# AberHu/TF-NAS

Hardware: AMD Instinct MI355X
Metric: supernet search images/sec (w-step + alpha-step) (higher is better)
Workload: dtype fp32

## Files before the change

tf-nas_amd/csrc/dwconv_kernels.hip:

```cpp
#include <cstring>
#include <type_traits>
#include "tfnas_dev.h"
#include "kernels.h"
#include "prof.h"
#include "efree.h"

__device__ __forceinline__ int floordiv(int a, int b) { return a >= 0 ? a / b : -((-a + b - 1) / b); }

__device__ __forceinline__ int xcd_first_tile() {
    const int gx = gridDim.x, bx = blockIdx.x;
    return (gx & 7) ? bx : (bx & 7) * (gx >> 3) + (bx >> 3);
}

template <int K, int DIL = 0>
__device__ __forceinline__ bool dw_locate(const TfnasCellDesc& d, int cy, int CC, int& g, int& c0) {
    for (g = 0; g < d.G; ++g) {
        if (d.g[g].k != K) continue;
        if (DIL != 0 && group_dil(d, g) != DIL) continue;
        const int t = (d.g[g].mcp + CC - 1) / CC;
        if (cy < t) {
            c0 = cy * CC;
            return true;
        }
        cy -= t;
    }
    return false;
}

struct DwSeg {
    int g, c0, mc, mcp, cs, woff;
};
template <int K, int DIL>
__device__ __forceinline__ bool dw_locate_seg(const TfnasCellDesc& d, int cy, int CC, DwSeg& sg) {
    for (int g = 0; g < d.G; ++g) {
        if (group_dil(d, g) != DIL) continue;
        const int n = group_nseg(d, g), q = d.g[g].mcp >> 2, mc = d.g[g].mc;
        int woff = 0;
        for (int s = 0; s < n; ++s) {
            const int ks = seg_k(d, g, s), lo = 4 * seg_quad0(q, n, s), hi = 4 * seg_quad0(q, n, s + 1);
            const int top = hi < mc ? hi : mc;
            if (ks == K) {
                const int t = (hi - lo + CC - 1) / CC;
                if (cy < t) {
                    sg = DwSeg{g, lo + cy * CC, top, hi, lo, woff};
                    return true;
                }
                cy -= t;
            }
            woff += (top - lo) * ks * ks;
        }
    }
    return false;
}

__device__ __forceinline__ void dw_flush_pair(f32x4 a, f32x4 b, float* red, int CC, int c0, int mcp, float* acc,
                                              bool = false) {
    const int tid = threadIdx.x, CQ = CC >> 2;
    __syncthreads();
    st4(red + tid * 8, a);
    st4(red + tid * 8 + 4, b);
    __syncthreads();
    if (tid < CC && c0 + tid < mcp) {
        const int cq = tid >> 2, comp = tid & 3;
        float s = 0.f, q = 0.f;
        for (int t = cq; t < 256; t += CQ) {
            s += red[t * 8 + comp];
            q += red[t * 8 + 4 + comp];
        }
        acc[2 * (size_t)(c0 + tid) + 0] = s;
        acc[2 * (size_t)(c0 + tid) + 1] = q;
    }
}

__device__ __forceinline__ void dw_flush_stats(f32x4 a, f32x4 b, float* lds, int CC, int c0, int mcp, int off, int M, float* part,
                                               int lane) {
    dw_flush_pair(a, b, lds, CC, c0, mcp, part + (size_t)lane * 2 * M + 2 * (size_t)off);
}

__device__ __forceinline__ void stage_weights(float* wts, const float* __restrict__ w, int KK, int CC, int c0, int mc, int cs = 0) {
    for (int idx = threadIdx.x; idx < KK * CC; idx += 256) {
        const int cl = idx % CC, t = idx / CC;
        wts[t * CC + cl] = (c0 + cl < mc) ? w[(size_t)(c0 + cl - cs) * KK + t] : 0.f;
    }
}

template <class FAddr, class FXf>
__device__ __forceinline__ void load_tile2(float* tile, int L0, int L1, int CC, int cq_shift,
                                           const float* __restrict__ src0, const float* __restrict__ src1, FAddr addr,
                                           FXf xf) {
    const int CQ = CC >> 2, total = L0 * L1 * CQ;
    const float inv_l1 = 1.f / (float)L1;
    for (int base = 0; base < total; base += 1024) {
        f32x4 v0[4], v1[4];
        int pix[4], cqv[4];
        bool ok[4];
#pragma unroll
        for (int u = 0; u < 4; ++u) {
            const int idx = base + u * 256 + threadIdx.x;
            pix[u] = idx >> cq_shift;
            cqv[u] = idx & (CQ - 1);
            const int r = (int)(((float)pix[u] + 0.5f) * inv_l1);
            const int c = pix[u] - r * L1;
            size_t a = 0;
            ok[u] = idx < total && addr(r, c, cqv[u], a);
            v0[u] = ok[u] ? ld4_nt(src0 + a) : zero4();
            v1[u] = ok[u] ? ld4_nt(src1 + a) : zero4();
        }
#pragma unroll
        for (int u = 0; u < 4; ++u) {
            const int idx = base + u * 256 + threadIdx.x;
            if (idx < total) st4(tile + pix[u] * CC + 4 * cqv[u], ok[u] ? xf(v0[u], v1[u], cqv[u]) : zero4());
        }
    }
}

template <class FAddr, class FXf>
__device__ __forceinline__ void load_tile(float* tile, int L0, int L1, int CC, int cq_shift, const float* __restrict__ src,
                                          FAddr addr, FXf xf) {
    const int CQ = CC >> 2, total = L0 * L1 * CQ;
    const float inv_l1 = 1.f / (float)L1;
    for (int base = 0; base < total; base += 1024) {
        f32x4 v[4];
        int pix[4], cqv[4];
        bool ok[4];
#pragma unroll
        for (int u = 0; u < 4; ++u) {
            const int idx = base + u * 256 + threadIdx.x;
            pix[u] = idx >> cq_shift;
            cqv[u] = idx & (CQ - 1);
            const int r = (int)(((float)pix[u] + 0.5f) * inv_l1);
            const int c = pix[u] - r * L1;
            size_t a = 0;
            ok[u] = idx < total && addr(r, c, cqv[u], a);
            v[u] = ok[u] ? ld4_nt(src + a) : zero4();
        }
#pragma unroll
        for (int u = 0; u < 4; ++u) {
            const int idx = base + u * 256 + threadIdx.x;
            if (idx < total) st4(tile + pix[u] * CC + 4 * cqv[u], ok[u] ? xf(v[u], cqv[u]) : zero4());
        }
    }
}

template <int K, int S, int ACT, int KQ, bool RAW = false, int DIL = 1>
__global__ __launch_bounds__(256, 4) void k_dw_fwd(TfnasCellDesc d, const float* __restrict__ E,
                                                   const float* __restrict__ x,
                                                   const double* __restrict__ stats1, float* __restrict__ D,
                                                   float* __restrict__ part, DwGeom gm) {
    extern __shared__ __attribute__((aligned(16))) float lds[];
    int g, c0, lane = blockIdx.x, cy = blockIdx.y;
    static_assert(DIL == 1 || (DIL == 2 && KQ == 0 && (K == 3 || K == 5)), "dilation 2: 3 x 3 / 5 x 5 from E or raw x");
    if (KQ > 0) efree_lane_chunk(lane, cy);
    DwSeg sg;
    if constexpr (KQ > 0) {
        if (!dw_locate<K, DIL>(d, cy, gm.CC, g, c0)) return;
        sg = DwSeg{g, c0, d.g[g].mc, d.g[g].mcp, 0, 0};
    } else {
        if (!dw_locate_seg<K, DIL>(d, cy, gm.CC, sg)) return;
        g = sg.g, c0 = sg.c0;
    }
    const int mc = sg.mc, mcp = sg.mcp, off = d.g[g].off;
    const int CC = gm.CC, CQ = CC >> 2, TH = gm.T0, TW = gm.T1;
    const int H = d.H, W = d.W, Ho = d.Ho, Wo = d.Wo, M = d.M;
    const int tid = threadIdx.x;
    const int IH = gm.L0, IW = gm.L1;

    const int tile_floats = max(IH * IW * CC, 2048);
    float* in_tile = lds;
    float* wts = lds + tile_floats;
    float2* cst = reinterpret_cast<float2*>(wts + K * K * CC);

    if constexpr (!RAW) {
    if (tid < CC)
        cst[tid] = (c0 + tid < mc) ? bn_consts(stats1 + 2 * (size_t)(off + c0 + tid), 1.0 / ((double)d.N * H * W), d.eps)
                                   : make_float2(0.f, 0.f);
    }
    stage_weights(wts, d.g[g].w_dw + sg.woff, K * K, CC, c0, mc, sg.cs);
    ExpandB<(KQ > 0 ? KQ : 2)> xb;
    if (KQ > 0) {
        __syncthreads();
        expand_b_load(xb, d.g[g].w_expand, d.ic, c0, mc, cst);
    }

    constexpr int KE = DIL * (K - 1) + 1, WIN = 3 * S + KE;
    const int nsw = TW >> 2, nstrips = TH * nsw;
    f32x4 ssum = zero4(), ssq = zero4();
    for (int t = KQ > 0 ? lane : xcd_first_tile(); t < gm.ntiles; t += gridDim.x) {
        const int tw = t % gm.tilesW, th = (t / gm.tilesW) % gm.tilesH, n = t / (gm.tilesW * gm.tilesH);
        const int ho0 = th * TH, wo0 = tw * TW;
        const int hi0 = ho0 * S - DIL * (K / 2), wi0 = wo0 * S - DIL * (K / 2);
        __syncthreads();
        if (KQ > 0) {
            const float inv_iw = 1.f / (float)IW;
            expand_tile<(KQ > 0 ? KQ : 2), ACT>(in_tile, IH * IW, CC, x, xb, [&](int p, size_t& a) {
                const int r = (int)(((float)p + 0.5f) * inv_iw), c = p - r * IW;
                const int hi = hi0 + r, wi = wi0 + c;
                a = ((size_t)(n * H + hi) * W + wi) * d.ic;
                return hi >= 0 && hi < H && wi >= 0 && wi < W;
            });
        } else if constexpr (RAW) {
            load_tile(in_tile, IH, IW, CC, gm.cq_shift, x,
                      [&](int r, int c, int cq, size_t& a) {
                          const int hi = hi0 + r, wi = wi0 + c;
                          a = ((size_t)(n * H + hi) * W + wi) * d.ic + c0 + 4 * cq;
                          return hi >= 0 && hi < H && wi >= 0 && wi < W && c0 + 4 * cq < mcp;
                      },
                      [&](f32x4 v, int) { return v; });
        } else
        load_tile(in_tile, IH, IW, CC, gm.cq_shift, E,
                  [&](int r, int c, int cq, size_t& a) {
                      const int hi = hi0 + r, wi = wi0 + c;
                      a = ((size_t)(n * H + hi) * W + wi) * M + off + c0 + 4 * cq;
                      return hi >= 0 && hi < H && wi >= 0 && wi < W && c0 + 4 * cq < mcp;
                  },
                  [&](f32x4 v, int cq) {
#pragma unroll
                      for (int j = 0; j < 4; ++j) {
                          const float2 c = cst[4 * cq + j];
                          v[j] = act_f<ACT>((v[j] - c.x) * c.y);
                      }
                      return v;
                  });
        __syncthreads();
        for (int item = tid; item < nstrips * CQ; item += 256) {
            const int cq = item & (CQ - 1), st = item >> gm.cq_shift;
            const int oh = st / nsw, ow0 = (st - oh * nsw) * 4;
            f32x4 acc[4] = {zero4(), zero4(), zero4(), zero4()};
#pragma unroll 1
            for (int ky = 0; ky < K; ++ky) {
                const float* rowp = in_tile + ((oh * S + ky * DIL) * IW + ow0 * S) * CC + 4 * cq;
                const float* wp = wts + ky * K * CC + 4 * cq;
                f32x4 win[WIN];
#pragma unroll
                for (int u = 0; u < WIN; ++u) win[u] = ld4(rowp + u * CC);
#pragma unroll
                for (int kx = 0; kx < K; ++kx) {
                    const f32x4 wv = ld4(wp + kx * CC);
#pragma unroll
                    for (int j = 0; j < 4; ++j) acc[j] += win[j * S + kx * DIL] * wv;
                }
            }
            const int ho = ho0 + oh;
            if (ho < Ho && c0 + 4 * cq < mcp) {
#pragma unroll
                for (int j = 0; j < 4; ++j) {
                    const int wo = wo0 + ow0 + j;
                    if (wo < Wo) {
                        st4_nt(D + (((size_t)(n * Ho + ho) * Wo + wo) * M + off + c0 + 4 * cq), acc[j]);
                        ssum += acc[j];
                        ssq += acc[j] * acc[j];
                    }
                }
            }
        }
    }
    dw_flush_stats(ssum, ssq, in_tile, CC, c0, mcp, off, M, part, lane);
}


template <int K, int S, int ACT, int KQ, bool RAW = false, int DIL = 1>
__global__ __launch_bounds__(256, 4) void k_dw_bwd_data(TfnasCellDesc d, const float* __restrict__ dZ,
                                                        const float* __restrict__ gate, const float* __restrict__ dpooled,
                                                        const float* __restrict__ D, const double* __restrict__ stats2,
                                                        const double* __restrict__ red2, const float* __restrict__ E,
                                                        const float* __restrict__ x,
                                                        const double* __restrict__ stats1, float* __restrict__ dEh,
                                                        float* __restrict__ part, DwGeom gm, int dx_accum) {
    extern __shared__ __attribute__((aligned(16))) float lds[];
    int g, c0, lane = blockIdx.x, cy = blockIdx.y;
    static_assert(DIL == 1 || (DIL == 2 && KQ == 0 && (K == 3 || K == 5)), "dilation 2: 3 x 3 / 5 x 5 from E or raw x");
    if (KQ > 0) efree_lane_chunk(lane, cy);
    DwSeg sg;
    if constexpr (KQ > 0) {
        if (!dw_locate<K, DIL>(d, cy, gm.CC, g, c0)) return;
        sg = DwSeg{g, c0, d.g[g].mc, d.g[g].mcp, 0, 0};
    } else {
        if (!dw_locate_seg<K, DIL>(d, cy, gm.CC, sg)) return;
        g = sg.g, c0 = sg.c0;
    }
    const int mc = sg.mc, mcp = sg.mcp, off = d.g[g].off;
    const int CC = gm.CC, CQ = CC >> 2, TIH = gm.T0, TIW = gm.T1;
    const int H = d.H, W = d.W, Ho = d.Ho, Wo = d.Wo, M = d.M;
    constexpr int PAD = DIL * (K / 2), KE = DIL * (K - 1) + 1;
    const int tid = threadIdx.x;
    const int OH = gm.L0, OW = gm.L1;

    const int tile_floats = max(OH * OW * CC, 2048);
    float* dd_tile = lds;
    float* wts = lds + tile_floats;
    f32x4* cst2 = reinterpret_cast<f32x4*>(wts + K * K * CC);
    float2* cst1 = reinterpret_cast<float2*>(cst2 + CC);

    fill_cst2(cst2, d, CC, c0, mc, off, stats2, red2);
    if constexpr (!RAW) {
    if (tid < CC)
        cst1[tid] = (c0 + tid < mc) ? bn_consts(stats1 + 2 * (size_t)(off + c0 + tid), 1.0 / ((double)d.N * H * W), d.eps)
                                    : make_float2(0.f, 0.f);
    }
    stage_weights(wts, d.g[g].w_dw + sg.woff, K * K, CC, c0, mc, sg.cs);
    float* eh_tile = reinterpret_cast<float*>(cst1 + CC);
    ExpandB<(KQ > 0 ? KQ : 2)> xb;
    if (KQ > 0) {
        __syncthreads();
        expand_b_load(xb, d.g[g].w_expand, d.ic, c0, mc, cst1);
    }

    const int nsw = TIW >> 2, nstrips = TIH * nsw;
    const bool has_se = d.g[g].se > 0;
    const float inv_hw = 1.f / (float)(Ho * Wo);
    f32x4 t1 = zero4(), t2 = zero4();
    for (int t = KQ > 0 ? lane : xcd_first_tile(); t < gm.ntiles; t += gridDim.x) {
        const int tw = t % gm.tilesW, th = (t / gm.tilesW) % gm.tilesH, n = t / (gm.tilesW * gm.tilesH);
        const int hi0 = th * TIH, wi0 = tw * TIW;
        const int oh0 = floordiv(hi0 + PAD - (KE - 1), S), ow0 = floordiv(wi0 + PAD - (KE - 1), S);
        __syncthreads();
        const int mycq = tid & (CQ - 1);
        f32x4 g4 = zero4(), dp4 = zero4();
        if (has_se && c0 + 4 * mycq < mcp) {
            g4 = ld4(gate + (size_t)n * M + off + c0 + 4 * mycq);
            dp4 = ld4(dpooled + (size_t)n * M + off + c0 + 4 * mycq) * splat4(inv_hw);
        }
        load_tile2(dd_tile, OH, OW, CC, gm.cq_shift, dZ, D,
                   [&](int r, int c, int cq, size_t& a) {
                       const int ho = oh0 + r, wo = ow0 + c;
                       a = ((size_t)(n * Ho + ho) * Wo + wo) * M + off + c0 + 4 * cq;
                       return ho >= 0 && ho < Ho && wo >= 0 && wo < Wo && c0 + 4 * cq < mcp;
                   },
                   [&](f32x4 v, f32x4 dv, int cq) { return bn2_dd<ACT>(cst2, 4 * cq, v, dv, has_se, g4, dp4); });
        if (KQ > 0) {
            const float inv_iw = 1.f / (float)TIW;
            expand_tile<(KQ > 0 ? KQ : 2), 2>(eh_tile, TIH * TIW, CC, x, xb, [&](int p, size_t& a) {
                const int r = (int)(((float)p + 0.5f) * inv_iw), c = p - r * TIW;
                const int hi = hi0 + r, wi = wi0 + c;
                a = ((size_t)(n * H + hi) * W + wi) * d.ic;
                return hi < H && wi < W;
            });
        }
        __syncthreads();

        for (int item = tid; item < nstrips * CQ; item += 256) {
            const int cq = item & (CQ - 1), st = item >> gm.cq_shift;
            const int ihp = st / nsw, iw0 = (st - ihp * nsw) * 4;
            const int half = (TIH + 1) >> 1;
            const int ih = (S == 2) ? (ihp < half ? 2 * ihp : 2 * (ihp - half) + 1) : ihp;
            const int hi = hi0 + ih;
            f32x4 acc[4] = {zero4(), zero4(), zero4(), zero4()};
            f32x4 ev[4];
#pragma unroll
            for (int j = 0; j < 4; ++j) {
                const int wi = wi0 + iw0 + j;
                const bool okj = hi < H && wi < W && c0 + 4 * cq < mcp;
                if constexpr (RAW) {
                    const size_t a = ((size_t)(n * H + hi) * W + wi) * d.ic + c0 + 4 * cq;
                    ev[j] = (okj && x) ? ld4_nt(x + a) : zero4();
                    if (okj && dx_accum) ev[j] += ld4_nt(dEh + a);
                }
                else if (KQ > 0) ev[j] = ld4(eh_tile + (ih * TIW + iw0 + j) * CC + 4 * cq);
                else ev[j] = okj ? ld4_nt(E + (((size_t)(n * H + hi) * W + wi) * M + off + c0 + 4 * cq)) : zero4();
            }
            if (S == 1) {
#pragma unroll 1
                for (int ky = 0; ky < K; ++ky) {
                    const int r = hi + PAD - ky * DIL - oh0;
                    const float* rowp = dd_tile + (r * OW + iw0) * CC + 4 * cq;
                    const float* wp = wts + ky * K * CC + 4 * cq;
                    f32x4 win[KE + 3];
#pragma unroll
                    for (int u = 0; u < KE + 3; ++u) win[u] = ld4(rowp + u * CC);
#pragma unroll
                    for (int kx = 0; kx < K; ++kx) {
                        const f32x4 wv = ld4(wp + kx * CC);
#pragma unroll
                        for (int j = 0; j < 4; ++j) acc[j] += win[j - kx * DIL + KE - 1] * wv;
                    }
                }
            } else {
                const int base = wi0 + iw0;
#pragma unroll 1
                for (int ky = 0; ky < K; ++ky) {
                    const int tt = hi + PAD - ky * DIL;
                    if (tt & 1) continue;
                    const int r = tt / 2 - oh0;
                    const float* wp = wts + ky * K * CC + 4 * cq;
#pragma unroll
                    for (int kx = 0; kx < K; ++kx) {
                        const f32x4 wv = ld4(wp + kx * CC);
#pragma unroll
                        for (int j = 0; j < 4; ++j) {
                            if ((j + PAD - kx * DIL) & 1) continue;
                            const int c = base / 2 + (j + PAD - kx * DIL) / 2 - ow0;
                            acc[j] += ld4(dd_tile + (r * OW + c) * CC + 4 * cq) * wv;
                        }
                    }
                }
            }
            if (hi < H && c0 + 4 * cq < mcp) {
#pragma unroll
                for (int j = 0; j < 4; ++j) {
                    const int wi = wi0 + iw0 + j;
                    if (wi < W) {
                        if constexpr (RAW) {
                            st4_nt(dEh + (((size_t)(n * H + hi) * W + wi) * d.ic + c0 + 4 * cq), acc[j] + ev[j]);
                        } else {
                        const size_t a = ((size_t)(n * H + hi) * W + wi) * M + off + c0 + 4 * cq;
                        const f32x4 e = ev[j];
                        f32x4 deh;
#pragma unroll
                        for (int q = 0; q < 4; ++q) {
                            const float2 c = cst1[4 * cq + q];
                            const float eh = KQ > 0 ? e[q] : (e[q] - c.x) * c.y;
                            deh[q] = acc[j][q] * act_d<ACT>(eh);
                            t1[q] += deh[q];
                            t2[q] += deh[q] * eh;
                        }
                        st4_nt(dEh + a, deh);
                        }
                    }
                }
            }
        }
    }
    if constexpr (!RAW) dw_flush_stats(t1, t2, dd_tile, CC, c0, mcp, off, M, part, lane);
}

template <int K, int S, int ACT, int KY0, int KR, bool RAW, int DIL>
__device__ __forceinline__ void dw_wgrad_rows(const TfnasCellDesc& d, const float* __restrict__ dZ,
                                              const float* __restrict__ gate, const float* __restrict__ dpooled,
                                              const float* __restrict__ D, const double* __restrict__ stats2,
                                              const double* __restrict__ red2, const float* __restrict__ E,
                                              const double* __restrict__ stats1, float* __restrict__ part,
                                              size_t out_size, const DwGeom& gm) {
    extern __shared__ __attribute__((aligned(16))) float lds[];
    DwSeg sg;
    if (!dw_locate_seg<K, DIL>(d, blockIdx.y, gm.CC, sg)) return;
    const int g = sg.g, c0 = sg.c0;
    const int mc = sg.mc, mcp = sg.mcp, off = d.g[g].off;
    size_t poff = sg.woff;
    for (int gg = 0; gg < g; ++gg) poff += group_dw_floats(d, gg);
    float* __restrict__ gw = part + (size_t)blockIdx.x * out_size + poff;
    const int CC = gm.CC, CQ = CC >> 2, TH = gm.T0, TW = gm.T1;
    const int H = d.H, W = d.W, Ho = d.Ho, Wo = d.Wo, M = d.M;
    const int tid = threadIdx.x;
    const int IH = gm.L0, IW = gm.L1;

    const int tile_floats = max(IH * IW * CC, 4 * KR * K * CC);
    float* in_tile = lds;
    f32x4* cst2 = reinterpret_cast<f32x4*>(lds + tile_floats);
    float2* cst1 = reinterpret_cast<float2*>(cst2 + CC);

    fill_cst2(cst2, d, CC, c0, mc, off, stats2, red2);
    if constexpr (!RAW) {
    if (tid < CC)
        cst1[tid] = (c0 + tid < mc) ? bn_consts(stats1 + 2 * (size_t)(off + c0 + tid), 1.0 / ((double)d.N * H * W), d.eps)
                                    : make_float2(0.f, 0.f);
    }

    constexpr int KE = DIL * (K - 1) + 1, WIN = 3 * S + KE;
    const int nsw = TW >> 2, nstrips = TH * nsw;
    const bool has_se = d.g[g].se > 0;
    const float inv_hw = 1.f / (float)(Ho * Wo);
    f32x4 wacc[KR * K];
#pragma unroll
    for (int u = 0; u < KR * K; ++u) wacc[u] = zero4();
    for (int t = xcd_first_tile(); t < gm.ntiles; t += gridDim.x) {
        const int tw = t % gm.tilesW, th = (t / gm.tilesW) % gm.tilesH, n = t / (gm.tilesW * gm.tilesH);
        const int ho0 = th * TH, wo0 = tw * TW;
        const int hi0 = ho0 * S - DIL * (K / 2), wi0 = wo0 * S - DIL * (K / 2);
        const int mycq = tid & (CQ - 1);
        f32x4 g4 = zero4(), dp4 = zero4();
        if (has_se && c0 + 4 * mycq < mcp) {
            g4 = ld4(gate + (size_t)n * M + off + c0 + 4 * mycq);
            dp4 = ld4(dpooled + (size_t)n * M + off + c0 + 4 * mycq) * splat4(inv_hw);
        }
        const int nitems = nstrips * CQ;
        auto item_ops = [&](int item, f32x4 (&dd)[4], f32x4 (&dv)[4], bool (&ok)[4]) {
            const int cq = item & (CQ - 1), st = item >> gm.cq_shift;
            const int oh = st / nsw, ow0 = (st - oh * nsw) * 4;
            const int ho = ho0 + oh;
#pragma unroll
            for (int j = 0; j < 4; ++j) {
                const int wo = wo0 + ow0 + j;
                ok[j] = ho < Ho && wo < Wo && c0 + 4 * cq < mcp;
                const size_t a = ((size_t)(n * Ho + ho) * Wo + wo) * M + off + c0 + 4 * cq;
                dd[j] = ok[j] ? ld4_nt(dZ + a) : zero4();
                dv[j] = ok[j] ? ld4_nt(D + a) : zero4();
            }
        };
        constexpr bool PF = KR == K;
        f32x4 pdd[PF ? 4 : 1], pdv[PF ? 4 : 1];
// ... 354 lines not shown
        return p;
    }
    dw_tile_plan(d, d.Ho, d.Wo, true, 2048, wout, false, p);
    return p;
}

template <bool TILE, int... Vs, class F>
static bool dw_dispatch_k(int k, int stride, int act, int v, F&& f) {
    bool hit = false;
    auto with_v = [&](auto K, auto S, auto A) {
        ((v == Vs ? (f(K, S, A, std::integral_constant<int, Vs>{}), hit = true) : false) || ...);
    };
    auto with_a = [&](auto K, auto S) {
        if (act == TFNAS_ACT_RELU) with_v(K, S, std::integral_constant<int, TFNAS_ACT_RELU>{});
        else if (act == TFNAS_ACT_SWISH) with_v(K, S, std::integral_constant<int, TFNAS_ACT_SWISH>{});
        else if constexpr (TILE) {
            if (act == TFNAS_ACT_RELU6) with_v(K, S, std::integral_constant<int, TFNAS_ACT_RELU6>{});
            else if (act == TFNAS_ACT_HSWISH) with_v(K, S, std::integral_constant<int, TFNAS_ACT_HSWISH>{});
        }
    };
    auto with_s = [&](auto K) {
        if (stride == 1) with_a(K, std::integral_constant<int, 1>{});
        else with_a(K, std::integral_constant<int, 2>{});
    };
    if (k == 3) with_s(std::integral_constant<int, 3>{});
    else if (k == 5) with_s(std::integral_constant<int, 5>{});
    else if constexpr (TILE) {
        if (k == 7) with_s(std::integral_constant<int, 7>{});
    }
    return hit;
}
template <int... Vs, class F>
static bool dw_dispatch(int k, int stride, int act, int v, F&& f) {
    return dw_dispatch_k<false, Vs...>(k, stride, act, v, f);
}
template <int... Vs, class F>
static bool dw_tile_dispatch(int k, int stride, int act, int v, F&& f) {
    return dw_dispatch_k<true, Vs...>(k, stride, act, v, f);
}
template <int... Vs, class F>
static bool dw_tile_dispatch_d(int k, int dil, int stride, int act, int v, F&& f) {
    if (dil == 1)
        return dw_tile_dispatch<Vs...>(k, stride, act, v, [&](auto K, auto S, auto A, auto V) {
            f(K, S, A, V, std::integral_constant<int, 1>{});
        });
    if (dil != 2 || (k != 3 && k != 5) || v != 0) return false;
    return dw_tile_dispatch<0>(k, stride, act, 0, [&](auto K, auto S, auto A, auto V) {
        if constexpr (K != 7) f(K, S, A, V, std::integral_constant<int, 2>{});
    });
}
constexpr int DW_WG = -1;
static int dws_variant(const DwPlan& p) { return p.fuse_wgrad ? DW_WG : p.kq ? p.kq : (int)p.pipe; }

static int dw_reduce_wgrad(const TfnasCellDesc& d, const float* wpart, int rows, size_t wout, hipStream_t s) {
    size_t poff = 0;
    for (int g = 0; g < d.G; ++g) {
        const int n = (int)group_dw_floats(d, g);
        const int rc = launch_reduce_rows(wpart + poff, rows, n, wout, nullptr, d.g[g].g_dw, s, wgrad_accum(d));
        if (rc) return rc;
        poff += n;
    }
    return 0;
}

int launch_dw_fwd(const TfnasCellDesc& d, const float* E, const float* x, const double* stats1, float* D,
                  double* stats2, float* part, hipStream_t s) {
    const bool raw = cell_noexpand(d);
    if (raw ? !x : (!E && (!efree_ic_ok(d.ic) || dw_tile_only(d)))) return TFNAS_EINVAL;
    const DwPlan p = dw_plan_fwd(d, !raw && E == nullptr, x != nullptr);
    for (int i = 0; i < DW_NK; ++i) {
        if (!p.chunks[i]) continue;
        const int kk = dw_slot_k(i), dil = dw_slot_dil(i);
        ProfScope _prof(TK_DW_FWD, s, d.G > 2);
        bool ok = false;
        if (p.fam != DW_TILE && i >= 2) return TFNAS_EINVAL;
        if (p.fam == DW_DIRECT) {
            const DwDirect gm = p.direct[i];
            ok = dw_dispatch<2, 4>(kk, d.stride, d.act, p.jw, [&](auto K, auto S, auto A, auto JW) {
                hipLaunchKernelGGL((k_dwd_fwd<K, S, A, JW>), dim3(gm.nwg), dim3(256), 0, s, d, E, stats1, D, part, gm);
            });
        } else if (p.fam == DW_RING) {
            const DwSlide gm = p.ring[i];
            const size_t shm = (size_t)(gm.RB * gm.L1 * gm.CCP + kk * kk * gm.CC + 2 * gm.CC) * sizeof(float);
            ok = dw_dispatch<0, 1, 6, 10>(kk, d.stride, d.act, dws_variant(p), [&](auto K, auto, auto A, auto V) {
                hipLaunchKernelGGL((k_dws_fwd<K, A, V == 1, V == 1 ? 0 : V>), dim3(p.rows * gm.chunks), dim3(256), shm, s, d, E,
                                   stats1, D, part, gm, V > 1 ? x : nullptr);
            });
        } else {
            const DwGeom gm = p.tile[i];
            const int tile = gm.L0 * gm.L1 * gm.CC > 2048 ? gm.L0 * gm.L1 * gm.CC : 2048;
            const size_t shm = (size_t)(tile + kk * kk * gm.CC + 2 * gm.CC) * sizeof(float);
            if (shm > 64 * 1024) return TFNAS_ERANGE;
            if (raw)
                ok = dw_tile_dispatch_d<0>(kk, dil, d.stride, TFNAS_ACT_RELU, 0, [&](auto K, auto S, auto, auto, auto DIL) {
                    hipLaunchKernelGGL((k_dw_fwd<K, S, TFNAS_ACT_RELU, 0, true, DIL>), dim3(p.rows, p.chunks[i]), dim3(256), shm, s,
                                       d, nullptr, x, nullptr, D, part, gm);
                });
            else
            ok = dw_tile_dispatch_d<0, 4, 6, 10>(kk, dil, d.stride, d.act, p.kq, [&](auto K, auto S, auto A, auto KQ, auto DIL) {
                if constexpr ((K != 7 && !act_tile_only(A)) || KQ == 0)
                    hipLaunchKernelGGL((k_dw_fwd<K, S, A, KQ, false, DIL>), dim3(p.rows, p.chunks[i]), dim3(256), shm, s, d, E, x,
                                       stats1, D, part, gm);
            });
        }
        if (!ok) return TFNAS_EINVAL;
    }
    return reduce_pair_rows(d, part, p.rows, stats2, s);
}

int launch_dw_bwd_data(const DwPlan& p, const TfnasCellDesc& d, const float* dZ, const float* gate, const float* dpooled,
                       const float* D, const double* stats2, const double* red2, const float* E, const float* x,
                       const double* stats1, float* dEh, double* red1, float* part, hipStream_t s, float* cb1) {
    if (cell_noexpand(d)) return TFNAS_EINVAL;
    if (!E && (!efree_ic_ok(d.ic) || dw_tile_only(d))) return TFNAS_EINVAL;
    const size_t wout = dw_wout_size(d);
    float* wpart = part + (((size_t)p.rows * 2 * d.M + 63) & ~(size_t)63);
    for (int i = 0; i < DW_NK; ++i) {
        if (!p.chunks[i]) continue;
        const int kk = dw_slot_k(i), dil = dw_slot_dil(i);
        ProfScope _prof(TK_DW_BWD_DATA, s, d.G > 2);
        bool ok = false;
        if (p.fam != DW_TILE && i >= 2) return TFNAS_EINVAL;
        if (p.fam == DW_DIRECT) {
            const DwDirect gm = p.direct[i];
            ok = dw_dispatch<2, 4, DW_WG>(kk, d.stride, d.act, p.fuse_wgrad ? DW_WG : p.jw, [&](auto K, auto S, auto A, auto V) {
                if constexpr (V == DW_WG)
                    hipLaunchKernelGGL((k_dwd_bwd<K, 2, A, 2, true>), dim3(gm.nwg), dim3(256), 0, s, d, dZ, gate, dpooled, D,
                                       stats2, red2, E, stats1, dEh, part, gm, wpart, wout);
                else
                    hipLaunchKernelGGL((k_dwd_bwd<K, S, A, V>), dim3(gm.nwg), dim3(256), 0, s, d, dZ, gate, dpooled, D, stats2,
                                       red2, E, stats1, dEh, part, gm);
            });
        } else if (p.fam == DW_RING) {
            const DwSlide gm = p.ring[i];
            size_t shm = (size_t)(gm.RB * gm.L1 * gm.CCP + kk * kk * gm.CC + 4 * gm.CC + 2 * gm.CC +
                                  (p.kq ? gm.TH * gm.TW * gm.CCP : 0)) * sizeof(float);
            if (p.fuse_wgrad && shm < (size_t)4 * kk * kk * gm.CC * sizeof(float)) shm = (size_t)4 * kk * kk * gm.CC * sizeof(float);
            ok = dw_dispatch<0, 1, 6, 10, DW_WG>(kk, d.stride, d.act, dws_variant(p), [&](auto K, auto, auto A, auto V) {
                if constexpr (V == DW_WG) {
                    if constexpr (K == 3)
                        hipLaunchKernelGGL((k_dws_bwd<K, A, false, 0, true>), dim3(p.rows * gm.chunks), dim3(256), shm, s, d, dZ,
                                           gate, dpooled, D, stats2, red2, E, stats1, dEh, part, gm, nullptr, wpart, wout);
                } else {
                    hipLaunchKernelGGL((k_dws_bwd<K, A, V == 1, V == 1 ? 0 : V>), dim3(p.rows * gm.chunks), dim3(256), shm, s, d,
                                       dZ, gate, dpooled, D, stats2, red2, E, stats1, dEh, part, gm, V > 1 ? x : nullptr);
                }
            });
        } else {
            const DwGeom gm = p.tile[i];
            const int tile = gm.L0 * gm.L1 * gm.CC > 2048 ? gm.L0 * gm.L1 * gm.CC : 2048;
            const size_t shm = (size_t)(tile + kk * kk * gm.CC + 4 * gm.CC + 2 * gm.CC + (p.kq ? gm.T0 * gm.T1 * gm.CC : 0)) *
                               sizeof(float);
            if (shm > 64 * 1024) return TFNAS_ERANGE;
            ok = dw_tile_dispatch_d<0, 4, 6, 10>(kk, dil, d.stride, d.act, p.kq, [&](auto K, auto S, auto A, auto KQ, auto DIL) {
                if constexpr ((K != 7 && !act_tile_only(A)) || KQ == 0)
                    hipLaunchKernelGGL((k_dw_bwd_data<K, S, A, KQ, false, DIL>), dim3(p.rows, p.chunks[i]), dim3(256), shm, s, d, dZ,
                                       gate, dpooled, D, stats2, red2, E, x, stats1, dEh, part, gm, 0);
            });
        }
        if (!ok) return TFNAS_EINVAL;
    }
    if (p.fuse_wgrad) {
        ProfScope _prof(TK_DW_WGRAD, s);
        const int rc = dw_reduce_wgrad(d, wpart, p.rows, wout, s);
        if (rc) return rc;
    }
    if (cb1) return launch_reduce_bn1(d, part, p.rows, stats1, red1, cb1, s);
    return launch_reduce_rows(part, p.rows, 2 * d.M, 2 * (size_t)d.M, red1, nullptr, s);
}

int launch_dw_bwd_dx(const TfnasCellDesc& d, const float* dZ, const float* gate, const float* dpooled, const float* D,
                     const double* stats2, const double* red2, const float* dres, float* dx, hipStream_t s, bool accum) {
    if (!cell_noexpand(d) || !dx) return TFNAS_EINVAL;
    if (accum && d.G != 1) return TFNAS_EINVAL;
    const DwPlan p = dw_plan_bwd_data(d, false, false);
    if (p.fam != DW_TILE) return TFNAS_EINVAL;
    for (int i = 0; i < DW_NK; ++i) {
        if (!p.chunks[i]) continue;
        const int kk = dw_slot_k(i), dil = dw_slot_dil(i);
        ProfScope _prof(TK_DW_BWD_DATA, s, false);
        const DwGeom gm = p.tile[i];
        const int tile = gm.L0 * gm.L1 * gm.CC > 2048 ? gm.L0 * gm.L1 * gm.CC : 2048;
        const size_t shm = (size_t)(tile + kk * kk * gm.CC + 4 * gm.CC + 2 * gm.CC) * sizeof(float);
        if (shm > 64 * 1024) return TFNAS_ERANGE;
        const bool ok = dw_tile_dispatch_d<0>(kk, dil, d.stride, d.act, 0, [&](auto K, auto S, auto A, auto, auto DIL) {
            hipLaunchKernelGGL((k_dw_bwd_data<K, S, A, 0, true, DIL>), dim3(p.rows, p.chunks[i]), dim3(256), shm, s, d, dZ, gate,
                               dpooled, D, stats2, red2, nullptr, dres, nullptr, dx, nullptr, gm, (int)accum);
        });
        if (!ok) return TFNAS_EINVAL;
    }
    return (int)hipGetLastError();
}

static constexpr int dw_wgrad_kr(int k, int stride, int dil) { return k == 7 ? 4 : (k == 5 && dil == 2 && stride == 1) ? 3 : k; }

int launch_dw_wgrad(const TfnasCellDesc& d, const float* dZ, const float* gate, const float* dpooled, const float* D,
                    const double* stats2, const double* red2, const float* E, const double* stats1, float* part,
                    hipStream_t s) {
    if (!dw_wgrad_row_fits(d)) return TFNAS_ERANGE;
    const DwPlan p = dw_plan_wgrad(d);
    const size_t wout = dw_wout_size(d);
    for (int i = 0; i < DW_NK; ++i) {
        if (!p.chunks[i]) continue;
        const int kk = dw_slot_k(i), dil = dw_slot_dil(i);
        ProfScope _prof(TK_DW_WGRAD, s);
        if (p.fam != DW_TILE && i >= 2) return TFNAS_EINVAL;
        if (p.fam == DW_DIRECT) {
            const DwDirect gm = p.direct[i];
            dw_dispatch<2, 4>(kk, d.stride, d.act, p.jw, [&](auto K, auto S, auto A, auto JW) {
                hipLaunchKernelGGL((k_dwd_wgrad<K, S, A, JW>), dim3(gm.nwg), dim3(256), 0, s, d, dZ, gate, dpooled, D, stats2,
                                   red2, E, stats1, part, wout, gm);
            });
        } else if (p.fam == DW_RING) {
            const DwSlide gm = p.ring[i];
            int ring = gm.RB * gm.L1 * gm.CCP;
            if (ring < 4 * kk * kk * gm.CC) ring = 4 * kk * kk * gm.CC;
            const size_t shm = (size_t)(ring + 4 * gm.CC + 2 * gm.CC) * sizeof(float);
            dw_dispatch<0, 1>(kk, d.stride, d.act, p.pipe, [&](auto K, auto, auto A, auto PIPE) {
                hipLaunchKernelGGL((k_dws_wgrad<K, A, PIPE == 1>), dim3(p.rows * gm.chunks), dim3(256), shm, s, d, dZ, gate,
                                   dpooled, D, stats2, red2, E, stats1, part, wout, gm);
            });
        } else {
            const DwGeom gm = p.tile[i];
            const int kr = dw_wgrad_kr(kk, d.stride, dil);
            int tile = gm.L0 * gm.L1 * gm.CC;
            if (tile < 4 * kr * kk * gm.CC) tile = 4 * kr * kk * gm.CC;
            const size_t shm = (size_t)(tile + 4 * gm.CC + 2 * gm.CC) * sizeof(float);
            if (shm > 64 * 1024) return TFNAS_ERANGE;
            if (cell_noexpand(d))
                dw_tile_dispatch_d<0>(kk, dil, d.stride, d.act, 0, [&](auto K, auto S, auto A, auto, auto DIL) {
                    constexpr int KR = dw_wgrad_kr(K, S, DIL);
                    hipLaunchKernelGGL((k_dw_wgrad<K, S, A, KR, true, DIL>), dim3(p.rows, p.chunks[i], (K + KR - 1) / KR), dim3(256),
                                       shm, s, d, dZ, gate, dpooled, D, stats2, red2, E, nullptr, part, wout, gm);
                });
            else
            dw_tile_dispatch_d<0>(kk, dil, d.stride, d.act, 0, [&](auto K, auto S, auto A, auto, auto DIL) {
                constexpr int KR = dw_wgrad_kr(K, S, DIL);
                hipLaunchKernelGGL((k_dw_wgrad<K, S, A, KR, false, DIL>), dim3(p.rows, p.chunks[i], (K + KR - 1) / KR), dim3(256), shm,
                                   s, d, dZ, gate, dpooled, D, stats2, red2, E, stats1, part, wout, gm);
            });
        }
    }
    const int rc = dw_reduce_wgrad(d, part, p.rows, wout, s);
    return rc ? rc : (int)hipGetLastError();
}
```

tf-nas_amd/csrc/efree.h:

```cpp
#pragma once
#include "tfnas_dev.h"

template <int KQ>
struct ExpandB {
    float b[2][KQ];
    float2 bc[2];
};

template <int KQ>
__device__ __forceinline__ void expand_b_load(ExpandB<KQ>& B, const float* __restrict__ w_expand, int ic, int c0, int mc,
                                              const float2* cst) {
    const int lane = threadIdx.x & 63, n = lane & 15, q = lane >> 4;
#pragma unroll
    for (int nt = 0; nt < 2; ++nt) {
        const int ch = c0 + 16 * nt + n;
#pragma unroll
        for (int kk = 0; kk < KQ; kk += 2) {
            float2 v = make_float2(0.f, 0.f);
            if (ch < mc) v = *reinterpret_cast<const float2*>(w_expand + (size_t)ch * ic + q * KQ + kk);
            B.b[nt][kk] = v.x;
            B.b[nt][kk + 1] = v.y;
        }
        B.bc[nt] = cst[16 * nt + n];
    }
}

template <int KQ, int OUT, class FLoc, class FDst>
__device__ __forceinline__ void expand_tile_to(int npix, const float* __restrict__ x, const ExpandB<KQ>& B, FLoc locate,
                                               FDst dst);
template <int KQ, int OUT, class FLoc>
__device__ __forceinline__ void expand_tile(float* tile, int npix, int CS, const float* __restrict__ x,
                                            const ExpandB<KQ>& B, FLoc locate) {
    expand_tile_to<KQ, OUT>(npix, x, B, locate, [&](int pix) { return tile + pix * CS; });
}
template <int KQ, int OUT, class FLoc, class FDst>
__device__ __forceinline__ void expand_tile_to(int npix, const float* __restrict__ x, const ExpandB<KQ>& B, FLoc locate,
                                               FDst dst) {
    constexpr int NB = KQ <= 4 ? 4 : (KQ <= 6 ? 3 : 2);
    const int lane = threadIdx.x & 63, wave = threadIdx.x >> 6, n = lane & 15, q = lane >> 4;
    const int nmt = (npix + 15) >> 4;
    for (int mt0 = wave; mt0 < nmt; mt0 += 4 * NB) {
        float a[NB][KQ];
        unsigned valid[NB];
#pragma unroll
        for (int b = 0; b < NB; ++b) {
            const int mt = mt0 + 4 * b;
            const int p = 16 * mt + n;
            size_t off = 0;
            const bool ok = mt < nmt && p < npix && locate(p, off);
#pragma unroll
            for (int kk = 0; kk < KQ; kk += 2) {
                float2 v = make_float2(0.f, 0.f);
                if (ok) v = *reinterpret_cast<const float2*>(x + off + q * KQ + kk);
                a[b][kk] = v.x;
                a[b][kk + 1] = v.y;
            }
            valid[b] = (unsigned)(__ballot(ok) & 0xffffull);
        }
#pragma unroll
        for (int b = 0; b < NB; ++b) {
            const int mt = mt0 + 4 * b;
            if (mt >= nmt) break;
            f32x4 acc0 = zero4(), acc1 = zero4();
#pragma unroll
            for (int kk = 0; kk < KQ; ++kk) {
                acc0 = __builtin_amdgcn_mfma_f32_16x16x4f32(a[b][kk], B.b[0][kk], acc0, 0, 0, 0);
                acc1 = __builtin_amdgcn_mfma_f32_16x16x4f32(a[b][kk], B.b[1][kk], acc1, 0, 0, 0);
            }
#pragma unroll
            for (int r = 0; r < 4; ++r) {
                const int pl = 4 * q + r, pix = 16 * mt + pl;
                if (pix < npix) {
                    float v0 = 0.f, v1 = 0.f;
                    if ((valid[b] >> pl) & 1u) {
                        v0 = (acc0[r] - B.bc[0].x) * B.bc[0].y;
                        v1 = (acc1[r] - B.bc[1].x) * B.bc[1].y;
                        if (OUT != 2) {
                            v0 = act_f<(OUT == 2 ? 0 : OUT)>(v0);
                            v1 = act_f<(OUT == 2 ? 0 : OUT)>(v1);
                        }
                    }
                    float* o = dst(pix);
                    o[n] = v0;
                    o[16 + n] = v1;
                }
            }
        }
    }
}

__device__ __forceinline__ void efree_lane_chunk(int& lane, int& cy) {
    const int gx = gridDim.x, chunks = gridDim.y, total = gx * chunks;
    const int L = blockIdx.x + gx * blockIdx.y;
    const int xcd = L & 7, rem = total & 7;
    const int V = xcd * (total >> 3) + (xcd < rem ? xcd : rem) + (L >> 3);
    lane = V / chunks;
    cy = V - lane * chunks;
}
```

Baseline: 4019.

## Prefetch next tile's expand inputs in registers across dwconv tile iterations

The fused expand-free depthwise forward and backward-data kernels now issue global loads of the next tile's input pixels into registers (ExpandA) before the current tile's compute finishes. The prefetched loads are consumed by MFMA expand at the start of the next iteration, and any leftover pixels go through the original loop. In backward, the expand compute is interleaved inside load_tile2 between its loads and stores. Occupancy for the 5x5 stride-2 forward is lowered to 3 workgroups per CU to make room for the prefetch registers, and a full-tile fast path drops the per-pixel validity checks.

After: 4060 (median of 3 runs). About the same (+1.0%).

```diff
diff --git a/tf-nas_amd/csrc/dwconv_kernels.hip b/tf-nas_amd/csrc/dwconv_kernels.hip
--- a/tf-nas_amd/csrc/dwconv_kernels.hip
+++ b/tf-nas_amd/csrc/dwconv_kernels.hip
@@ -6,6 +6,19 @@
 #include "efree.h"
 
 __device__ __forceinline__ int floordiv(int a, int b) { return a >= 0 ? a / b : -((-a + b - 1) / b); }
+
+constexpr int dw_efree_nr(int K, int S, int KQ, bool fwd) {
+    return !fwd ? 2 : KQ > 6 ? 2 : S == 2 ? (K == 5 ? 7 : 5) : (K == 5 ? 5 : 4);
+}
+__device__ __forceinline__ int dw_per_tile_s(int v) {
+    asm volatile("" : "+s"(v));
+    return v;
+}
+__device__ __forceinline__ int dw_per_tile_v(int v) {
+    asm volatile("" : "+v"(v));
+    return v;
+}
+constexpr int dw_fwd_wgs(int K, int S, int KQ) { return KQ > 0 && K == 5 && S == 2 ? 3 : 4; }
 
 __device__ __forceinline__ int xcd_first_tile() {
     const int gx = gridDim.x, bx = blockIdx.x;
@@ -84,10 +97,10 @@
     }
 }
 
-template <class FAddr, class FXf>
+template <class FAddr, class FXf, class FMid>
 __device__ __forceinline__ void load_tile2(float* tile, int L0, int L1, int CC, int cq_shift,
                                            const float* __restrict__ src0, const float* __restrict__ src1, FAddr addr,
-                                           FXf xf) {
+                                           FXf xf, FMid mid, int tid) {
     const int CQ = CC >> 2, total = L0 * L1 * CQ;
     const float inv_l1 = 1.f / (float)L1;
     for (int base = 0; base < total; base += 1024) {
@@ -96,7 +109,7 @@
         bool ok[4];
 #pragma unroll
         for (int u = 0; u < 4; ++u) {
-            const int idx = base + u * 256 + threadIdx.x;
+            const int idx = base + u * 256 + tid;
             pix[u] = idx >> cq_shift;
             cqv[u] = idx & (CQ - 1);
             const int r = (int)(((float)pix[u] + 0.5f) * inv_l1);
@@ -106,9 +119,10 @@
             v0[u] = ok[u] ? ld4_nt(src0 + a) : zero4();
             v1[u] = ok[u] ? ld4_nt(src1 + a) : zero4();
         }
+        if (base == 0) mid();
 #pragma unroll
         for (int u = 0; u < 4; ++u) {
-            const int idx = base + u * 256 + threadIdx.x;
+            const int idx = base + u * 256 + tid;
             if (idx < total) st4(tile + pix[u] * CC + 4 * cqv[u], ok[u] ? xf(v0[u], v1[u], cqv[u]) : zero4());
         }
     }
@@ -143,10 +157,10 @@
 }
 
 template <int K, int S, int ACT, int KQ, bool RAW = false, int DIL = 1>
-__global__ __launch_bounds__(256, 4) void k_dw_fwd(TfnasCellDesc d, const float* __restrict__ E,
-                                                   const float* __restrict__ x,
-                                                   const double* __restrict__ stats1, float* __restrict__ D,
-                                                   float* __restrict__ part, DwGeom gm) {
+__global__ __launch_bounds__(256, dw_fwd_wgs(K, S, KQ)) void k_dw_fwd(TfnasCellDesc d, const float* __restrict__ E,
+                                                                      const float* __restrict__ x,
+                                                                      const double* __restrict__ stats1, float* __restrict__ D,
+                                                                      float* __restrict__ part, DwGeom gm) {
     extern __shared__ __attribute__((aligned(16))) float lds[];
     int g, c0, lane = blockIdx.x, cy = blockIdx.y;
     static_assert(DIL == 1 || (DIL == 2 && KQ == 0 && (K == 3 || K == 5)), "dilation 2: 3 x 3 / 5 x 5 from E or raw x");
@@ -185,19 +199,37 @@
     constexpr int KE = DIL * (K - 1) + 1, WIN = 3 * S + KE;
     const int nsw = TW >> 2, nstrips = TH * nsw;
     f32x4 ssum = zero4(), ssq = zero4();
+    constexpr int NR = dw_efree_nr(K, S, KQ, true);
+    ExpandA<(KQ > 0 ? KQ : 2), NR> xa;
+    auto x_loc = [&](int t) {
+        const int tw = t % gm.tilesW, th = (t / gm.tilesW) % gm.tilesH, n = t / (gm.tilesW * gm.tilesH);
+        const int hi0 = th * TH * S - DIL * (K / 2), wi0 = tw * TW * S - DIL * (K / 2), ic = d.ic;
+        const float inv_iw = 1.f / (float)IW;
+        return [=](int p, size_t& a) {
+            const int r = (int)(((float)p + 0.5f) * inv_iw), c = p - r * IW;
+            const int hi = hi0 + r, wi = wi0 + c;
+            a = ((size_t)(n * H + hi) * W + wi) * ic;
+            return hi >= 0 && hi < H && wi >= 0 && wi < W;
+        };
+    };
+    auto x_issue = [&](int t) {
+        const int tid_t = dw_per_tile_v(tid);
+        expand_issue(xa, __builtin_amdgcn_readfirstlane(tid_t >> 6), dw_per_tile_s(IH * IW), x, x_loc(t), tid_t);
+    };
+    if constexpr (KQ > 0) {
+        if (lane < gm.ntiles) x_issue(lane);
+    }
     for (int t = KQ > 0 ? lane : xcd_first_tile(); t < gm.ntiles; t += gridDim.x) {
         const int tw = t % gm.tilesW, th = (t / gm.tilesW) % gm.tilesH, n = t / (gm.tilesW * gm.tilesH);
         const int ho0 = th * TH, wo0 = tw * TW;
         const int hi0 = ho0 * S - DIL * (K / 2), wi0 = wo0 * S - DIL * (K / 2);
         __syncthreads();
-        if (KQ > 0) {
-            const float inv_iw = 1.f / (float)IW;
-            expand_tile<(KQ > 0 ? KQ : 2), ACT>(in_tile, IH * IW, CC, x, xb, [&](int p, size_t& a) {
-                const int r = (int)(((float)p + 0.5f) * inv_iw), c = p - r * IW;
-                const int hi = hi0 + r, wi = wi0 + c;
-                a = ((size_t)(n * H + hi) * W + wi) * d.ic;
-                return hi >= 0 && hi < H && wi >= 0 && wi < W;
-            });
+        if constexpr (KQ > 0) {
+            const int npix = dw_per_tile_s(IH * IW), tid_t = dw_per_tile_v(tid);
+            auto dst = [&](int pix) { return in_tile + pix * 32; };
+            expand_compute<KQ, NR, ACT>(xa, __builtin_amdgcn_readfirstlane(tid_t >> 6), npix, xb, dst, tid_t);
+            expand_tile_to<KQ, ACT>(npix, x, xb, x_loc(t), dst, NR, tid_t);
+            if (t + (int)gridDim.x < gm.ntiles) x_issue(t + gridDim.x);
         } else if constexpr (RAW) {
             load_tile(in_tile, IH, IW, CC, gm.cq_shift, x,
                       [&](int r, int c, int cq, size_t& a) {
@@ -309,6 +341,26 @@
     const bool has_se = d.g[g].se > 0;
     const float inv_hw = 1.f / (float)(Ho * Wo);
     f32x4 t1 = zero4(), t2 = zero4();
+    constexpr int NR = dw_efree_nr(K, S, KQ, false);
+    ExpandA<(KQ > 0 ? KQ : 2), NR> xa;
+    auto x_loc = [&](int t) {
+        const int tw = t % gm.tilesW, th = (t / gm.tilesW) % gm.tilesH, n = t / (gm.tilesW * gm.tilesH);
+        const int hi0 = th * TIH, wi0 = tw * TIW, ic = d.ic;
+        const float inv_iw = 1.f / (float)TIW;
+        return [=](int p, size_t& a) {
+            const int r = (int)(((float)p + 0.5f) * inv_iw), c = p - r * TIW;
+            const int hi = hi0 + r, wi = wi0 + c;
+            a = ((size_t)(n * H + hi) * W + wi) * ic;
+            return hi < H && wi < W;
+        };
+    };
+    auto x_issue = [&](int t) {
+        const int tid_t = dw_per_tile_v(tid);
+        expand_issue(xa, __builtin_amdgcn_readfirstlane(tid_t >> 6), dw_per_tile_s(TIH * TIW), x, x_loc(t), tid_t);
+    };
+    if constexpr (KQ > 0) {
+        if (lane < gm.ntiles) x_issue(lane);
+    }
     for (int t = KQ > 0 ? lane : xcd_first_tile(); t < gm.ntiles; t += gridDim.x) {
         const int tw = t % gm.tilesW, th = (t / gm.tilesW) % gm.tilesH, n = t / (gm.tilesW * gm.tilesH);
         const int hi0 = th * TIH, wi0 = tw * TIW;
@@ -320,21 +372,24 @@
             g4 = ld4(gate + (size_t)n * M + off + c0 + 4 * mycq);
             dp4 = ld4(dpooled + (size_t)n * M + off + c0 + 4 * mycq) * splat4(inv_hw);
         }
+        int tid_l = tid;
+        if constexpr (KQ > 0) tid_l = dw_per_tile_v(tid);
         load_tile2(dd_tile, OH, OW, CC, gm.cq_shift, dZ, D,
                    [&](int r, int c, int cq, size_t& a) {
                        const int ho = oh0 + r, wo = ow0 + c;
                        a = ((size_t)(n * Ho + ho) * Wo + wo) * M + off + c0 + 4 * cq;
                        return ho >= 0 && ho < Ho && wo >= 0 && wo < Wo && c0 + 4 * cq < mcp;
                    },
-                   [&](f32x4 v, f32x4 dv, int cq) { return bn2_dd<ACT>(cst2, 4 * cq, v, dv, has_se, g4, dp4); });
-        if (KQ > 0) {
-            const float inv_iw = 1.f / (float)TIW;
-            expand_tile<(KQ > 0 ? KQ : 2), 2>(eh_tile, TIH * TIW, CC, x, xb, [&](int p, size_t& a) {
-                const int r = (int)(((float)p + 0.5f) * inv_iw), c = p - r * TIW;
-                const int hi = hi0 + r, wi = wi0 + c;
-                a = ((size_t)(n * H + hi) * W + wi) * d.ic;
-                return hi < H && wi < W;
-            });
+                   [&](f32x4 v, f32x4 dv, int cq) { return bn2_dd<ACT>(cst2, 4 * cq, v, dv, has_se, g4, dp4); },
+                   [&]() {
+                       if constexpr (KQ > 0) {
+                           const int tid_t = dw_per_tile_v(tid);
+                           expand_compute<KQ, NR, 2>(xa, __builtin_amdgcn_readfirstlane(tid_t >> 6), dw_per_tile_s(TIH * TIW), xb,
+                                                     [&](int pix) { return eh_tile + pix * 32; }, tid_t);
+                       }
+                   }, tid_l);
+        if constexpr (KQ > 0) {
+            if (t + (int)gridDim.x < gm.ntiles) x_issue(t + gridDim.x);
         }
         __syncthreads();
 
@@ -995,6 +1050,7 @@
             const size_t shm = (size_t)(tile + kk * kk * gm.CC + 4 * gm.CC + 2 * gm.CC + (p.kq ? gm.T0 * gm.T1 * gm.CC : 0)) *
                                sizeof(float);
             if (shm > 64 * 1024) return TFNAS_ERANGE;
+            if (p.kq && gm.T0 * gm.T1 > 64 * dw_efree_nr(kk, d.stride, p.kq, false)) return TFNAS_ERANGE;
             ok = dw_tile_dispatch_d<0, 4, 6, 10>(kk, dil, d.stride, d.act, p.kq, [&](auto K, auto S, auto A, auto KQ, auto DIL) {
                 if constexpr ((K != 7 && !act_tile_only(A)) || KQ == 0)
                     hipLaunchKernelGGL((k_dw_bwd_data<K, S, A, KQ, false, DIL>), dim3(p.rows, p.chunks[i]), dim3(256), shm, s, d, dZ,
diff --git a/tf-nas_amd/csrc/efree.h b/tf-nas_amd/csrc/efree.h
--- a/tf-nas_amd/csrc/efree.h
+++ b/tf-nas_amd/csrc/efree.h
@@ -25,68 +25,102 @@
     }
 }
 
+template <int KQ, int NR>
+struct ExpandA {
+    float a[NR][KQ];
+    unsigned valid[NR];
+};
+
+template <int KQ, int NR, class FLoc>
+__device__ __forceinline__ void expand_issue(ExpandA<KQ, NR>& A, int mt0, int npix, const float* __restrict__ x, FLoc locate,
+                                             int tid) {
+    const int lane = tid & 63, n = lane & 15, q = lane >> 4;
+    const int nmt = (npix + 15) >> 4;
+#pragma unroll
+    for (int b = 0; b < NR; ++b) {
+        const int mt = mt0 + 4 * b;
+        const int p = 16 * mt + n;
+        size_t off = 0;
+        const bool ok = mt < nmt && p < npix && locate(p, off);
+#pragma unroll
+        for (int kk = 0; kk < KQ; kk += 2) {
+            float2 v = make_float2(0.f, 0.f);
+            if (ok) v = *reinterpret_cast<const float2*>(x + off + q * KQ + kk);
+            A.a[b][kk] = v.x;
+            A.a[b][kk + 1] = v.y;
+        }
+        A.valid[b] = (unsigned)(__ballot(ok) & 0xffffull);
+    }
+}
+
+template <int KQ, int NR, int OUT, class FDst>
+__device__ __forceinline__ void expand_compute(const ExpandA<KQ, NR>& A, int mt0, int npix, const ExpandB<KQ>& B, FDst dst,
+                                               int tid) {
+    const int lane = tid & 63, n = lane & 15, q = lane >> 4;
+    const int nmt = (npix + 15) >> 4;
+#pragma unroll
+    for (int b = 0; b < NR; ++b) {
+        const int mt = mt0 + 4 * b;
+        if (mt >= nmt) break;
+        f32x4 acc0 = zero4(), acc1 = zero4();
+#pragma unroll
+        for (int kk = 0; kk < KQ; ++kk) {
+            acc0 = __builtin_amdgcn_mfma_f32_16x16x4f32(A.a[b][kk], B.b[0][kk], acc0, 0, 0, 0);
+            acc1 = __builtin_amdgcn_mfma_f32_16x16x4f32(A.a[b][kk], B.b[1][kk], acc1, 0, 0, 0);
+        }
+        if (16 * mt + 16 <= npix && A.valid[b] == 0xffffu) {
+#pragma unroll
+            for (int r = 0; r < 4; ++r) {
+                float v0 = (acc0[r] - B.bc[0].x) * B.bc[0].y;
+                float v1 = (acc1[r] - B.bc[1].x) * B.bc[1].y;
+                if (OUT != 2) {
+                    v0 = act_f<(OUT == 2 ? 0 : OUT)>(v0);
+                    v1 = act_f<(OUT == 2 ? 0 : OUT)>(v1);
+                }
+                float* o = dst(16 * mt + 4 * q + r);
+                o[n] = v0;
+                o[16 + n] = v1;
+            }
+            continue;
+        }
+#pragma unroll
+        for (int r = 0; r < 4; ++r) {
+            const int pl = 4 * q + r, pix = 16 * mt + pl;
+            if (pix < npix) {
+                float v0 = 0.f, v1 = 0.f;
+                if ((A.valid[b] >> pl) & 1u) {
+                    v0 = (acc0[r] - B.bc[0].x) * B.bc[0].y;
+                    v1 = (acc1[r] - B.bc[1].x) * B.bc[1].y;
+                    if (OUT != 2) {
+                        v0 = act_f<(OUT == 2 ? 0 : OUT)>(v0);
+                        v1 = act_f<(OUT == 2 ? 0 : OUT)>(v1);
+                    }
+                }
+                float* o = dst(pix);
+                o[n] = v0;
+                o[16 + n] = v1;
+            }
+        }
+    }
+}
+
 template <int KQ, int OUT, class FLoc, class FDst>
 __device__ __forceinline__ void expand_tile_to(int npix, const float* __restrict__ x, const ExpandB<KQ>& B, FLoc locate,
-                                               FDst dst);
+                                               FDst dst, int mt_first = 0, int tid_or_neg = -1) {
+    constexpr int NB = KQ <= 4 ? 4 : (KQ <= 6 ? 3 : 2);
+    const int tid = tid_or_neg < 0 ? (int)threadIdx.x : tid_or_neg;
+    const int wave = __builtin_amdgcn_readfirstlane(tid >> 6);
+    const int nmt = (npix + 15) >> 4;
+    for (int mt0 = wave + 4 * mt_first; mt0 < nmt; mt0 += 4 * NB) {
+        ExpandA<KQ, NB> A;
+        expand_issue(A, mt0, npix, x, locate, tid);
+        expand_compute<KQ, NB, OUT>(A, mt0, npix, B, dst, tid);
+    }
+}
 template <int KQ, int OUT, class FLoc>
 __device__ __forceinline__ void expand_tile(float* tile, int npix, int CS, const float* __restrict__ x,
                                             const ExpandB<KQ>& B, FLoc locate) {
     expand_tile_to<KQ, OUT>(npix, x, B, locate, [&](int pix) { return tile + pix * CS; });
-}
-template <int KQ, int OUT, class FLoc, class FDst>
-__device__ __forceinline__ void expand_tile_to(int npix, const float* __restrict__ x, const ExpandB<KQ>& B, FLoc locate,
-                                               FDst dst) {
-    constexpr int NB = KQ <= 4 ? 4 : (KQ <= 6 ? 3 : 2);
-    const int lane = threadIdx.x & 63, wave = threadIdx.x >> 6, n = lane & 15, q = lane >> 4;
-    const int nmt = (npix + 15) >> 4;
-    for (int mt0 = wave; mt0 < nmt; mt0 += 4 * NB) {
-        float a[NB][KQ];
-        unsigned valid[NB];
-#pragma unroll
-        for (int b = 0; b < NB; ++b) {
-            const int mt = mt0 + 4 * b;
-            const int p = 16 * mt + n;
-            size_t off = 0;
-            const bool ok = mt < nmt && p < npix && locate(p, off);
-#pragma unroll
-            for (int kk = 0; kk < KQ; kk += 2) {
-                float2 v = make_float2(0.f, 0.f);
-                if (ok) v = *reinterpret_cast<const float2*>(x + off + q * KQ + kk);
-                a[b][kk] = v.x;
-                a[b][kk + 1] = v.y;
-            }
-            valid[b] = (unsigned)(__ballot(ok) & 0xffffull);
-        }
-#pragma unroll
-        for (int b = 0; b < NB; ++b) {
-            const int mt = mt0 + 4 * b;
-            if (mt >= nmt) break;
-            f32x4 acc0 = zero4(), acc1 = zero4();
-#pragma unroll
-            for (int kk = 0; kk < KQ; ++kk) {
-                acc0 = __builtin_amdgcn_mfma_f32_16x16x4f32(a[b][kk], B.b[0][kk], acc0, 0, 0, 0);
-                acc1 = __builtin_amdgcn_mfma_f32_16x16x4f32(a[b][kk], B.b[1][kk], acc1, 0, 0, 0);
-            }
-#pragma unroll
-            for (int r = 0; r < 4; ++r) {
-                const int pl = 4 * q + r, pix = 16 * mt + pl;
-                if (pix < npix) {
-                    float v0 = 0.f, v1 = 0.f;
-                    if ((valid[b] >> pl) & 1u) {
-                        v0 = (acc0[r] - B.bc[0].x) * B.bc[0].y;
-                        v1 = (acc1[r] - B.bc[1].x) * B.bc[1].y;
-                        if (OUT != 2) {
-                            v0 = act_f<(OUT == 2 ? 0 : OUT)>(v0);
-                            v1 = act_f<(OUT == 2 ? 0 : OUT)>(v1);
-                        }
-                    }
-                    float* o = dst(pix);
-                    o[n] = v0;
-                    o[16 + n] = v1;
-                }
-            }
-        }
-    }
 }
 
 __device__ __forceinline__ void efree_lane_chunk(int& lane, int& cy) {
```
